# xiaochuanle/MECAT

Hardware: AMD Instinct MI355X
Metric: candidate overlaps/sec (higher is better)
Workload: dtype int32

## Files before the change

### mecat_amd/csrc/seed_cand.hip

```cpp
#include "seed_defs.h"
#include "seed_replay.h"

struct CandLds {
    int t_loc[2 * SM + 10];
    int t_seed[2 * SM + 10];
};

__device__ __forceinline__ int seg_find(const uint32_t* __restrict__ seg_id, int nseg, uint32_t seg) {
    int lo = 0, hi = nseg;
    while (lo < hi) {
        int mid = (lo + hi) >> 1;
        if (seg_id[mid] < seg) lo = mid + 1; else hi = mid;
    }
    return (lo < nseg && seg_id[lo] == seg) ? lo : -1;
}

__device__ __forceinline__ bool ddf_find(int dloc, int dseed, double cutoff) {
    float r = (float)dloc / ((float)dseed * 10.0f) - 1.0f;
    return (double)fabsf(r) < cutoff;
}

__device__ __forceinline__ bool ddf_find_quarter(int dloc, int dseed) {
    return (int)(2 * dloc > __mul24(15, dseed)) & (int)(2 * dloc < __mul24(25, dseed));
}

__device__ __forceinline__ int write_lane(int v, int l, int old) {
    asm volatile("s_mov_b32 m0, %2\n\tv_writelane_b32 %0, %1, m0" : "+v"(old) : "s"(v), "s"(l));
    return old;
}

__global__ __launch_bounds__(WAVE) __attribute__((amdgpu_waves_per_eu(7, 7))) void seed_cand(SeedArrays AF, SeedArrays AB, const mhip_offset_t* __restrict__ ref_offs, const uint32_t* __restrict__ ref_blk, int ref_nreads,
                                                  int ref_start_id, const mhip_offset_t* __restrict__ roffs, ReadSel sel, int ib,
                                                  int reads_start_id, mhip_params P, mhip_candidate* __restrict__ out,
                                                  int32_t* __restrict__ out_counts, unsigned long long* __restrict__ counters) {
    extern __shared__ __attribute__((aligned(16))) int smem[];
    const int lane = lane_id();
    const int r = blockIdx.x;
    const bool big = P.maxc > MAXC_LDS;
    int* clist = big ? (int*)(out + (size_t)r * P.maxc) : smem;
    CandLds* T = (CandLds*)(smem + (big ? 0 : P.maxc * 12));
    auto cl_ld = [&](int i) -> int { return big ? __hip_atomic_load(clist + i, __ATOMIC_RELAXED, __HIP_MEMORY_SCOPE_AGENT) : clist[i]; };
    auto cl_st = [&](int i, int v) { if (big) __hip_atomic_store(clist + i, v, __ATOMIC_RELAXED, __HIP_MEMORY_SCOPE_AGENT); else clist[i] = v; };
    const int rid = sel_rid(sel, ib + r);
    const int read_id = rid + reads_start_id;
    const int read_size = roffs[rid].size;
    const int MAXC = P.maxc;
    const double cutoff = P.ddfs_cutoff;
    int ncand = 0;

    for (int strand = 0; strand < 2; ++strand) {
        const int s = 2 * r + strand;
        const SeedArrays& A = AF.fused[s] ? AF : AB;
        const uint64_t hb = A.hit_base[s];
        const int nseg = (int)A.nseg[s];
        const int ng = (int)A.ngated[s];
        if (A.strand_hits[s] == 0) continue;
        uint32_t* ent = A.ent + hb;
        uint32_t* fin = A.ent_fin + hb;
        const uint32_t* seg_id = A.seg_id + hb;
        const uint32_t* seg_start = A.seg_start + hb;
        int32_t* seg_score = A.seg_score + hb;
        const uint32_t* gated = A.gated + hb;
#define SEG_LIST(g) (((seg_score[g] & OVF_FLAG) ? fin : ent) + seg_start[g])
#define SEG_SCORE(g) (seg_score[g] & ~OVF_FLAG)
#define SET_SCORE(g, v) seg_score[g] = (seg_score[g] & OVF_FLAG) | (v)

        int g_n = 0, seg_n = 0, segm1_n = -1;
        uint32_t st_n = 0, stm1_n = 0;
        auto prefetch = [&](int gi) {
            g_n = (int)gated[gi];
            seg_n = (int)seg_id[g_n];
            st_n = seg_start[g_n];
            segm1_n = g_n > 0 ? (int)seg_id[g_n - 1] : -1;
            stm1_n = g_n > 0 ? seg_start[g_n - 1] : 0u;
        };
        if (ng > 0) prefetch(0);
        for (int gi = 0; gi < ng; ++gi) {
            const int g = g_n, seg = seg_n, segm1 = segm1_n;
            const uint32_t st_g = st_n, st_gm1 = stm1_n;
            if (gi + 1 < ng) prefetch(gi + 1);
#ifdef CAND_STATS
            if (lane == 0) atomicAdd(&counters[9], 1ull);
#endif
            const int raw_g = seg_score[g];
            int s_k = raw_g & ~OVF_FLAG;
            if (s_k == 0) continue;
#ifdef CAND_STATS
            if (lane == 0) atomicAdd(&counters[10], 1ull);
#endif
            int start_loc = seg * ZV;
            int loc = 0, raw_gm1 = 0;
            const bool has_left = seg > 0 && g > 0 && segm1 == seg - 1;
            if (has_left) { raw_gm1 = seg_score[g - 1]; loc = raw_gm1 & ~OVF_FLAG; }
            if (loc > 0) start_loc = (seg - 1) * ZV;
            const int n1 = loc > 0 ? min(loc, SM) : 0, n2 = min(s_k, SM);
            const int k = n1 + n2;
            const uint32_t* list_g = ((raw_g & OVF_FLAG) ? fin : ent) + st_g;
            const uint32_t* list_gm1 = ((raw_gm1 & OVF_FLAG) ? fin : ent) + st_gm1;
            __syncthreads();
            for (int i = lane; i < k; i += 64) {
                uint32_t e = i < n1 ? list_gm1[i] : list_g[i - n1];
                T->t_loc[i] = ent_loc(e) + ((i >= n1 && loc > 0) ? ZV : 0);
                T->t_seed[i] = ent_seed(e);
            }
            __syncthreads();
            const int i0 = lane, i1 = lane + 64;
            const int l0 = i0 < k ? T->t_loc[i0] : 0, d0 = i0 < k ? T->t_seed[i0] : 0;
            const int l1 = i1 < k ? T->t_loc[i1] : 0, d1 = i1 < k ? T->t_seed[i1] : 0;
            int temp0 = d0, temp1 = d1, sc0 = 0, sc1 = 0;
            const int k0 = min(k, 64);
            int in0 = 0, in1 = 0;
            auto vote_loops = [&](auto ddf) {
                for (int j = 1; j < k0; ++j) {
                    const int lj = __builtin_amdgcn_readlane(l0, j), dj = __builtin_amdgcn_readlane(d0, j);
                    const int ds = dj - d0, dl = lj - l0;
                    const bool v0 = (i0 < j) & (temp0 != dj) & (ds > 0) & (dl > 0) & (dl < read_size) & ddf(dl, ds);
                    sc0 += v0 ? 1 : 0;
                    temp0 = v0 ? dj : temp0;
                    in0 = write_lane(__popcll(__builtin_amdgcn_ballot_w64(v0)), j, in0);
                }
                for (int j = 64; j < k; ++j) {
                    const int lj = __builtin_amdgcn_readlane(l1, j - 64), dj = __builtin_amdgcn_readlane(d1, j - 64);
                    const int ds0 = dj - d0, dl0 = lj - l0, ds1 = dj - d1, dl1 = lj - l1;
                    const bool v0 = (temp0 != dj) & (ds0 > 0) & (dl0 > 0) & (dl0 < read_size) & ddf(dl0, ds0);
                    const bool v1 = (i1 < j) & (temp1 != dj) & (ds1 > 0) & (dl1 > 0) & (dl1 < read_size) & ddf(dl1, ds1);
                    sc0 += v0 ? 1 : 0;
                    temp0 = v0 ? dj : temp0;
                    sc1 += v1 ? 1 : 0;
                    temp1 = v1 ? dj : temp1;
                    in1 = write_lane(__popcll(__builtin_amdgcn_ballot_w64(v0)) + __popcll(__builtin_amdgcn_ballot_w64(v1)), j - 64, in1);
                }
            };
            if (cutoff == 0.25) vote_loops([](int dloc, int dseed) { return ddf_find_quarter(dloc, dseed); });
            else vote_loops([&](int dloc, int dseed) { return (dloc > 0) & (dseed > 0) & ddf_find(dloc, dseed, cutoff); });
            sc0 += in0;
            sc1 += in1;
            int mv = max(i0 < k ? sc0 : -1, i1 < k ? sc1 : -1);
            for (int o = 32; o > 0; o >>= 1) mv = max(mv, __shfl_xor(mv, o));
            const int maxval = mv;
#ifdef CAND_STATS
            if (lane == 0 && maxval < 5) atomicAdd(&counters[11], 1ull);
            if (lane == 0) atomicAdd(&counters[12], (unsigned long long)k);
#endif
            if (maxval < 5) continue;
            const uint64_t eq0 = __ballot(i0 < k && sc0 == maxval), eq1 = __ballot(i1 < k && sc1 == maxval);
            const int maxi = eq0 ? __ffsll((unsigned long long)eq0) - 1 : 64 + __ffsll((unsigned long long)eq1) - 1;
            const int rep = __popcll(eq0) + __popcll(eq1) - 1;
            int rep_loc;
            if (rep == maxval) {
                rep_loc = maxi;
            } else {
                const int lm = T->t_loc[maxi], dm = T->t_seed[maxi];
                bool q0 = false, q1 = false;
                if (i0 < k) {
                    if (i0 < maxi) q0 = dm - d0 > 0 && lm - l0 > 0 && lm - l0 < read_size && ddf_find(lm - l0, dm - d0, cutoff);
                    else if (i0 == maxi) q0 = true;
                    else q0 = d0 - dm > 0 && l0 - lm > 0 && l0 - lm <= read_size && ddf_find(l0 - lm, d0 - dm, cutoff);
                }
                if (i1 < k) {
                    if (i1 < maxi) q1 = dm - d1 > 0 && lm - l1 > 0 && lm - l1 < read_size && ddf_find(lm - l1, dm - d1, cutoff);
                    else if (i1 == maxi) q1 = true;
                    else q1 = d1 - dm > 0 && l1 - lm > 0 && l1 - lm <= read_size && ddf_find(l1 - lm, d1 - dm, cutoff);
                }
                const uint64_t s0m = __ballot(q0), s1m = __ballot(q1);
                const uint64_t z0 = __ballot(q0 && l0 != 0), z1 = __ballot(q1 && l1 != 0);
                if (z0) rep_loc = __ffsll((unsigned long long)z0) - 1;
                else if (z1) rep_loc = 64 + __ffsll((unsigned long long)z1) - 1;
                else if (s1m) rep_loc = 64 + (63 - __clzll((unsigned long long)s1m));
                else rep_loc = 63 - __clzll((unsigned long long)s0m);
            }
            const int vote = rep_loc < 64 ? __shfl(sc0, rep_loc) : __shfl(sc1, rep_loc - 64);
            if (vote < 2 * P.min_kmer_match + 2) continue;
            const int loc_seed = T->t_seed[rep_loc];
            const int loc_list = start_loc + T->t_loc[rep_loc];
            int sid = read_id_lookup(ref_offs, ref_nreads, ref_blk, loc_list);
            const int sstart = ref_offs[sid].offset, ssize = ref_offs[sid].size;
            const int send = sstart + ssize + 1;
            sid += ref_start_id;
            if (sid > read_id) continue;
            if (sid == read_id) {
                int u_k = sstart / ZV;
                int gg = seg_find(seg_id, nseg, (uint32_t)u_k);
                if (gg >= 0) {
                    const int lim = sstart % ZV, cnt = min(SEG_SCORE(gg), SM);
                    uint32_t* L = SEG_LIST(gg);
                    uint32_t e = lane < cnt ? L[lane] : 0;
                    bool keep = lane < cnt && ent_loc(e) < lim;
                    uint64_t km = __ballot(keep);
                    int dstp = __popcll(km & ((1ull << lane) - 1ull));
                    __syncthreads();
                    if (keep) L[dstp] = (L[dstp] & 0xFFFFu) | (e & 0xFFFF0000u);
                    __syncthreads();
                    if (lane == 0) SET_SCORE(gg, __popcll(km));
                }
                ++u_k;
                const int kend = send / ZV;
                {
                    int lo = 0, hi = nseg;
                    while (lo < hi) { int mid = (lo + hi) >> 1; if ((int)seg_id[mid] < u_k) lo = mid + 1; else hi = mid; }
                    for (int x = lo + lane; x < nseg && (int)seg_id[x] < kend; x += 64) SET_SCORE(x, 0);
                }
                const int tail_seg = max(u_k, kend);
                gg = seg_find(seg_id, nseg, (uint32_t)tail_seg);
                __syncthreads();
                if (gg >= 0) {
                    const int lim = send % ZV, cnt = min(SEG_SCORE(gg), SM);
                    uint32_t* L = SEG_LIST(gg);
                    uint32_t e = lane < cnt ? L[lane] : 0;
                    bool keep = lane < cnt && ent_loc(e) > lim;
                    uint64_t km = __ballot(keep);
                    int dstp = __popcll(km & ((1ull << lane) - 1ull));
                    __syncthreads();
                    if (keep) L[dstp] = (L[dstp] & 0xFFFFu) | (e & 0xFFFF0000u);
                    __syncthreads();
                    if (lane == 0) SET_SCORE(gg, __popcll(km));
                }
                __syncthreads();
                continue;
            }
            const int loc2 = (loc_seed - 1) * BC;
            const int left1 = loc_list - sstart + MHIP_KMER_SIZE - 1, right1 = send - loc_list;
            const int left2 = loc2 + MHIP_KMER_SIZE - 1, right2 = read_size - loc2;
            const int num1 = left1 > left2 ? left2 : left1, num2 = right1 > right2 ? right2 : right1;
            if (num1 + num2 < P.min_kmer_dist) continue;
            int seedcount = 0;
            {
                int nlb = (num1 + ZV - 1) / ZV;
                const int lowest = max(0, seg - nlb);
                for (int x = g - 1; x >= 0 && (int)seg_id[x] >= lowest; --x) {
                    const int sc = SEG_SCORE(x);
                    if (sc <= 0) continue;
                    const int sl = (int)seg_id[x] * ZV, scnt = min(sc, SM);
                    bool ok = false;
                    if (lane < scnt) {
                        uint32_t e = SEG_LIST(x)[lane];
                        ok = fabs((double)(loc_list - sl - ent_loc(e)) / ((double)((loc_seed - ent_seed(e)) * BC) * 1.0) - 1.0) < cutoff;
                    }
                    const int agree = __popcll(__ballot(ok));
                    seedcount += agree;
                    if (agree * 1.0 / scnt > 0.4) { if (lane == 0) SET_SCORE(x, 0); }
                    __syncthreads();
                }
                int nrb = (num2 + ZV - 1) / ZV;
                const int highest = seg + nrb;
                for (int x = g + 1; x < nseg && (int)seg_id[x] <= highest; ++x) {
                    const int sc = SEG_SCORE(x);
                    if (sc <= 0) continue;
                    const int sl = (int)seg_id[x] * ZV, scnt = min(sc, SM);
                    bool ok = false;
                    if (lane < scnt) {
                        uint32_t e = SEG_LIST(x)[lane];
                        ok = fabs((double)(sl + ent_loc(e) - loc_list) / ((double)((ent_seed(e) - loc_seed) * BC) * 1.0) - 1.0) < cutoff;
                    }
                    const int agree = __popcll(__ballot(ok));
                    seedcount += agree;
                    if (agree * 1.0 / scnt > 0.4) { if (lane == 0) SET_SCORE(x, 0); }
                    __syncthreads();
                }
            }
            const int cscore = vote + seedcount;
            int ge = 0;
            for (int i = lane; i < ncand; i += 64) ge += cl_ld(i * 12 + 6) >= cscore ? 1 : 0;
            for (int o = 32; o > 0; o >>= 1) ge += __shfl_xor(ge, o);
            const int pos = ge;
            const int last_src = (ncand < MAXC) ? ncand - 1 : ncand - 2;
            __syncthreads();
            for (int top = last_src; top >= pos; top -= 64) {
                const int i = top - lane;
                int v[12];
                if (i >= pos) {
#pragma unroll
                    for (int q = 0; q < 12; ++q) v[q] = cl_ld(i * 12 + q);
                }
                __syncthreads();
                if (i >= pos) {
#pragma unroll
                    for (int q = 0; q < 12; ++q) cl_st((i + 1) * 12 + q, v[q]);
                }
                __syncthreads();
            }
            if (pos < MAXC && lane == 0) {
                const int cv[12] = {loc_list - sstart, loc2, left1, left2, right1, right2, cscore, num1, num2, sid, sstart, strand};
#pragma unroll
                for (int q = 0; q < 12; ++q) cl_st(pos * 12 + q, cv[q]);
            }
            if (ncand < MAXC) ++ncand;
            __syncthreads();
        }
#undef SEG_LIST
#undef SEG_SCORE
#undef SET_SCORE
    }
    __syncthreads();
    int* o = (int*)(out + (size_t)r * MAXC);
    if (!big)
        for (int i = lane; i < ncand * 12; i += 64) o[i] = clist[i];
    if (lane == 0) {
        out_counts[r] = ncand;
        atomicAdd(&counters[2], (unsigned long long)ncand);
    }
}

int seed_run_cand(const SeedBatch& b) {
    mhip_ctx* c = b.c;
    const mhip_params* P = b.P;
    const size_t lds = sizeof(int) * 12 * (size_t)(P->maxc > MAXC_LDS ? 0 : P->maxc) + sizeof(CandLds);
    LAUNCH(c, "seed_cand", seed_cand, b.nr, WAVE, lds, b.F, b.B, (const mhip_offset_t*)b.ref->d_offs, (const uint32_t*)b.ref->d_blk2read,
           b.ref->num_reads, b.ref->start_read_id, (const mhip_offset_t*)b.reads->d_offs, b.sel, b.ib, b.reads->start_read_id, *P, b.d_out,
           b.d_counts, (unsigned long long*)c->d_counters);
    return 0;
}
```

### mecat_amd/csrc/seed_replay.h

```cpp
#pragma once

#include "seed_defs.h"

__device__ __forceinline__ int sweep_reach(int L) { return (L + MHIP_KMER_SIZE - 1 + ZV - 1) / ZV + 1; }

__device__ __forceinline__ bool ddf_insert(int dloc, int dseed, double cutoff) {
    float r = (float)dloc / ((float)dseed * 10.0f);
    return fabs((double)r - 1.0) < cutoff;
}

__device__ void replay_overflow(const uint32_t* __restrict__ ev, int c, uint32_t* __restrict__ fin, uint16_t* __restrict__ esc,
                                double cutoff, int* score_out) {
    const int lane = lane_id();
    int loc = 0, seed = 0;
    if (lane < SM) { const uint32_t e0 = ev[lane]; loc = ent_loc(e0); seed = ent_seed(e0); }
    if (lane < SM) esc[lane] = (uint16_t)(lane + 1);
    int score = SM;
    int e = SM;
    auto is_chain = [&]() {
        const int nl = __shfl_down(loc, 1), ns = __shfl_down(seed, 1);
        return (bool)__all(lane >= SM - 1 || (ns - seed > 0 && nl - loc == (ns - seed) * BC));
    };
    bool chain = is_chain();
    while (e < c) {
        if (chain) {
            const int lloc = __builtin_amdgcn_readlane(loc, SM - 1), lseed = __builtin_amdgcn_readlane(seed, SM - 1);
            int nb = c;
            for (int i0 = e; i0 < c && nb == c; i0 += 64) {
                const int i = i0 + lane;
                bool bad = false;
                if (i < c) {
                    const uint32_t b = ev[i];
                    int pl = lloc, ps = lseed;
                    if (i > e) { const uint32_t a = ev[i - 1]; pl = ent_loc(a); ps = ent_seed(a); }
                    const int ds = ent_seed(b) - ps, dl = ent_loc(b) - pl;
                    bad = !(ds > 0 && dl == ds * BC);
                }
                const unsigned long long bm = __ballot(bad);
                if (bm) nb = i0 + __builtin_ctzll(bm);
            }
            if (nb > e) {
                for (int x = e + lane; x < nb; x += 64) esc[x] = (uint16_t)(score + (x - e) + 1);
                score += nb - e;
                if (lane == SM - 1) { const uint32_t le = ev[nb - 1]; loc = ent_loc(le); seed = ent_seed(le); }
                e = nb;
                if (e >= c) break;
            }
        }
        const uint32_t ne = ev[e];
        const int nloc = ent_loc(ne), nseed = ent_seed(ne);
        ++score;
        const int myloc = lane < SM ? loc : nloc, myseed = lane < SM ? seed : nseed;
        int sc = 0;
        for (int i = 0; i < SM; ++i) {
            const int li = __builtin_amdgcn_readlane(myloc, i), si = __builtin_amdgcn_readlane(myseed, i);
            const bool pass = lane > i && lane <= SM && myseed - si > 0 && myloc - li > 0 && ddf_insert(myloc - li, myseed - si, cutoff);
            const uint64_t b = __ballot(pass);
            sc += pass ? 1 : 0;
            if (lane == i) sc += __popcll(b);
        }
        const int v = lane <= SM ? sc : 0x7fffffff;
        int m = v;
        for (int o = 32; o > 0; o >>= 1) m = min(m, __shfl_xor(m, o));
        const int minval = m;
        const int mini = __ffsll((unsigned long long)__ballot(v == m)) - 1;
        if (minval == SM) {
            if (lane == SM - 1) { loc = nloc; seed = nseed; }
        } else if (minval < SM && mini < SM) {
            const int sl = __shfl_down(myloc, 1), ss = __shfl_down(myseed, 1);
            if (lane >= mini && lane < SM) { loc = sl; seed = ss; }
            --score;
        }
        if (lane == 0) esc[e] = (uint16_t)score;
        ++e;
        chain = is_chain();
    }
    if (lane < SM) fin[lane] = ((uint32_t)loc << 16) | ((uint32_t)seed & 0xFFFFu);
    *score_out = score;
}

__device__ __forceinline__ int read_id_from_offset(const mhip_offset_t* __restrict__ a, int n, int offset) {
    int left = 0, right = n - 1, mid = (left + right) / 2;
    if (a[right].offset < offset) return right;
    while (left <= right) {
        int o = a[mid].offset, z = a[mid].size;
        if (o <= offset && o + z > offset) return mid;
        if (o + z <= offset) left = mid + 1;
        else right = mid - 1;
        mid = (left + right) / 2;
    }
    return mid;
}

__device__ __forceinline__ int read_id_lookup(const mhip_offset_t* __restrict__ a, int n, const uint32_t* __restrict__ blk, int offset) {
    if (offset >= 0) {
        int r = (int)blk[offset >> 10];
        while (r + 1 < n && a[r].offset + a[r].size <= offset) ++r;
        const int o = a[r].offset, z = a[r].size;
        if (o <= offset && o + z > offset) return r;
    }
    return read_id_from_offset(a, n, offset);
}

__device__ __forceinline__ bool subjects_all_higher(const RefReads& R, uint32_t seg, int rid, int own_end) {
    const int lo = (int)((seg > 0 ? seg - 1u : 0u) * (uint32_t)ZV);
    if (R.same_volume) return lo >= own_end;
    return read_id_lookup(R.offs, R.nreads, R.blk, lo) + R.start_id > rid + R.reads_start_id;
}
```

Before: 7.212 million.

## Batch gated-segment metadata per wave and parallelize neighbor-segment sweep across lanes

```diff
diff --git a/mecat_amd/csrc/seed_cand.hip b/mecat_amd/csrc/seed_cand.hip
--- a/mecat_amd/csrc/seed_cand.hip
+++ b/mecat_amd/csrc/seed_cand.hip
@@ -1,5 +1,7 @@
 #include "seed_defs.h"
 #include "seed_replay.h"
+
+#define SWEEP_G 8
 
 struct CandLds {
     int t_loc[2 * SM + 10];
@@ -35,7 +37,7 @@
                                                   int32_t* __restrict__ out_counts, unsigned long long* __restrict__ counters) {
     extern __shared__ __attribute__((aligned(16))) int smem[];
     const int lane = lane_id();
-    const int r = blockIdx.x;
+    const int r = (int)gridDim.x - 1 - (int)blockIdx.x;
     const bool big = P.maxc > MAXC_LDS;
     int* clist = big ? (int*)(out + (size_t)r * P.maxc) : smem;
     CandLds* T = (CandLds*)(smem + (big ? 0 : P.maxc * 12));
@@ -64,34 +66,47 @@
 #define SEG_LIST(g) (((seg_score[g] & OVF_FLAG) ? fin : ent) + seg_start[g])
 #define SEG_SCORE(g) (seg_score[g] & ~OVF_FLAG)
 #define SET_SCORE(g, v) seg_score[g] = (seg_score[g] & OVF_FLAG) | (v)
-
-        int g_n = 0, seg_n = 0, segm1_n = -1;
-        uint32_t st_n = 0, stm1_n = 0;
-        auto prefetch = [&](int gi) {
-            g_n = (int)gated[gi];
-            seg_n = (int)seg_id[g_n];
-            st_n = seg_start[g_n];
-            segm1_n = g_n > 0 ? (int)seg_id[g_n - 1] : -1;
-            stm1_n = g_n > 0 ? seg_start[g_n - 1] : 0u;
-        };
-        if (ng > 0) prefetch(0);
+#define HAS_LEFT 0x40000000
+
+        int gv = 0, segv = 0, scv = 0, scm1v = 0;
+        uint32_t stv = 0, stm1v = 0;
+        bool stale = true;
         for (int gi = 0; gi < ng; ++gi) {
-            const int g = g_n, seg = seg_n, segm1 = segm1_n;
-            const uint32_t st_g = st_n, st_gm1 = stm1_n;
-            if (gi + 1 < ng) prefetch(gi + 1);
+            const int gj = gi & 63;
+            if (gj == 0) {
+                gv = segv = 0;
+                stv = stm1v = 0;
+                if (gi + lane < ng) {
+                    gv = (int)gated[gi + lane];
+                    segv = (int)seg_id[gv];
+                    stv = seg_start[gv];
+                    const int segm1 = gv > 0 ? (int)seg_id[gv - 1] : -1;
+                    if (segv > 0 && gv > 0 && segm1 == segv - 1) { segv |= HAS_LEFT; stm1v = seg_start[gv - 1]; }
+                }
+                stale = true;
+            }
+            if (stale) {
+                scv = scm1v = 0;
+                if (gi - gj + lane < ng) {
+                    scv = seg_score[gv];
+                    if (segv & HAS_LEFT) scm1v = seg_score[gv - 1];
+                }
+                stale = false;
+            }
 #ifdef CAND_STATS
             if (lane == 0) atomicAdd(&counters[9], 1ull);
 #endif
-            const int raw_g = seg_score[g];
+            const int raw_g = __builtin_amdgcn_readlane(scv, gj);
             int s_k = raw_g & ~OVF_FLAG;
             if (s_k == 0) continue;
 #ifdef CAND_STATS
             if (lane == 0) atomicAdd(&counters[10], 1ull);
 #endif
+            const int g = __builtin_amdgcn_readlane(gv, gj), seg = __builtin_amdgcn_readlane(segv, gj) & ~HAS_LEFT;
+            const uint32_t st_g = (uint32_t)__builtin_amdgcn_readlane((int)stv, gj), st_gm1 = (uint32_t)__builtin_amdgcn_readlane((int)stm1v, gj);
+            const int raw_gm1 = __builtin_amdgcn_readlane(scm1v, gj);
+            const int loc = raw_gm1 & ~OVF_FLAG;
             int start_loc = seg * ZV;
-            int loc = 0, raw_gm1 = 0;
-            const bool has_left = seg > 0 && g > 0 && segm1 == seg - 1;
-            if (has_left) { raw_gm1 = seg_score[g - 1]; loc = raw_gm1 & ~OVF_FLAG; }
             if (loc > 0) start_loc = (seg - 1) * ZV;
             const int n1 = loc > 0 ? min(loc, SM) : 0, n2 = min(s_k, SM);
             const int k = n1 + n2;
@@ -170,10 +185,11 @@
                 else rep_loc = 63 - __clzll((unsigned long long)s0m);
             }
             const int vote = rep_loc < 64 ? __shfl(sc0, rep_loc) : __shfl(sc1, rep_loc - 64);
+            const int loc_seed = __builtin_amdgcn_readfirstlane(T->t_seed[rep_loc]);
+            const int loc_list = start_loc + __builtin_amdgcn_readfirstlane(T->t_loc[rep_loc]);
+            const int blk_r = loc_list >= 0 ? (int)ref_blk[loc_list >> 10] : 0;
             if (vote < 2 * P.min_kmer_match + 2) continue;
-            const int loc_seed = T->t_seed[rep_loc];
-            const int loc_list = start_loc + T->t_loc[rep_loc];
-            int sid = read_id_lookup(ref_offs, ref_nreads, ref_blk, loc_list);
+            int sid = read_id_lookup_from(ref_offs, ref_nreads, blk_r, loc_list);
             const int sstart = ref_offs[sid].offset, ssize = ref_offs[sid].size;
             const int send = sstart + ssize + 1;
             sid += ref_start_id;
@@ -216,6 +232,7 @@
                     if (lane == 0) SET_SCORE(gg, __popcll(km));
                 }
                 __syncthreads();
+                stale = true;
                 continue;
             }
             const int loc2 = (loc_seed - 1) * BC;
@@ -225,38 +242,57 @@
             if (num1 + num2 < P.min_kmer_dist) continue;
             int seedcount = 0;
             {
-                int nlb = (num1 + ZV - 1) / ZV;
+                const int nlb = (num1 + ZV - 1) / ZV, nrb = (num2 + ZV - 1) / ZV;
                 const int lowest = max(0, seg - nlb);
-                for (int x = g - 1; x >= 0 && (int)seg_id[x] >= lowest; --x) {
-                    const int sc = SEG_SCORE(x);
-                    if (sc <= 0) continue;
-                    const int sl = (int)seg_id[x] * ZV, scnt = min(sc, SM);
-                    bool ok = false;
-                    if (lane < scnt) {
-                        uint32_t e = SEG_LIST(x)[lane];
-                        ok = fabs((double)(loc_list - sl - ent_loc(e)) / ((double)((loc_seed - ent_seed(e)) * BC) * 1.0) - 1.0) < cutoff;
+                const int highest = seg + nrb;
+                const bool lside = lane < 32;
+                uint64_t more = ~0ull;
+                for (int c = 0; more; ++c) {
+                    const int x = lside ? g - 1 - 32 * c - lane : g + 1 + 32 * c + (lane - 32);
+                    int id = -1, raw = 0;
+                    uint32_t st = 0;
+                    if (((more >> lane) & 1) && x >= 0 && x < nseg) { id = (int)seg_id[x]; raw = seg_score[x]; st = seg_start[x]; }
+                    const bool in = id >= 0 && (lside ? id >= lowest : id <= highest);
+                    const uint64_t inm = __builtin_amdgcn_ballot_w64(in);
+                    more = ((uint32_t)inm == 0xFFFFFFFFu ? 0xFFFFFFFFull : 0ull) | ((uint32_t)(inm >> 32) == 0xFFFFFFFFu ? 0xFFFFFFFF00000000ull : 0ull);
+                    const int scnt = min(raw & ~OVF_FLAG, SM);
+                    const uint64_t live = __builtin_amdgcn_ballot_w64(in && (raw & ~OVF_FLAG) > 0);
+                    int agv = 0;
+                    uint64_t m = live;
+                    while (m) {
+                        uint32_t e[SWEEP_G];
+                        uint64_t p = m;
+#pragma unroll
+                        for (int q = 0; q < SWEEP_G; ++q) {
+                            const bool has = p != 0;
+                            const int j = has ? __builtin_ctzll(p) : 0;
+                            p &= p - 1;
+                            const int rj = __builtin_amdgcn_readlane(raw, j);
+                            const uint32_t* L = ((rj & OVF_FLAG) ? fin : ent) + (uint32_t)__builtin_amdgcn_readlane((int)st, j);
+                            e[q] = 0;
+                            if (has && lane < min(rj & ~OVF_FLAG, SM)) e[q] = L[lane];
+                        }
+#pragma unroll
+                        for (int q = 0; q < SWEEP_G; ++q) {
+                            if (m) {
+                                const int j = __builtin_ctzll(m);
+                                m &= m - 1;
+                                const int sl = __builtin_amdgcn_readlane(id, j) * ZV, sc = __builtin_amdgcn_readlane(scnt, j);
+                                const int l = ent_loc(e[q]), sd = ent_seed(e[q]);
+                                const int dl = j < 32 ? loc_list - sl - l : sl + l - loc_list;
+                                const int ds = j < 32 ? loc_seed - sd : sd - loc_seed;
+                                const bool ok = lane < sc && fabs((double)dl / ((double)(ds * BC) * 1.0) - 1.0) < cutoff;
+                                const int agree = __popcll(__builtin_amdgcn_ballot_w64(ok));
+                                seedcount += agree;
+                                agv = write_lane(agree, j, agv);
+                            }
+                        }
                     }
-                    const int agree = __popcll(__ballot(ok));
-                    seedcount += agree;
-                    if (agree * 1.0 / scnt > 0.4) { if (lane == 0) SET_SCORE(x, 0); }
-                    __syncthreads();
-                }
-                int nrb = (num2 + ZV - 1) / ZV;
-                const int highest = seg + nrb;
-                for (int x = g + 1; x < nseg && (int)seg_id[x] <= highest; ++x) {
-                    const int sc = SEG_SCORE(x);
-                    if (sc <= 0) continue;
-                    const int sl = (int)seg_id[x] * ZV, scnt = min(sc, SM);
-                    bool ok = false;
-                    if (lane < scnt) {
-                        uint32_t e = SEG_LIST(x)[lane];
-                        ok = fabs((double)(sl + ent_loc(e) - loc_list) / ((double)((ent_seed(e) - loc_seed) * BC) * 1.0) - 1.0) < cutoff;
-                    }
-                    const int agree = __popcll(__ballot(ok));
-                    seedcount += agree;
-                    if (agree * 1.0 / scnt > 0.4) { if (lane == 0) SET_SCORE(x, 0); }
-                    __syncthreads();
-                }
+                    const bool zero = ((live >> lane) & 1) && agv * 1.0 / scnt > 0.4;
+                    if (zero) seg_score[x] = raw & OVF_FLAG;
+                    stale |= __builtin_amdgcn_ballot_w64(zero) != 0;
+                }
+                if (stale) __syncthreads();
             }
             const int cscore = vote + seedcount;
             int ge = 0;
@@ -290,6 +326,7 @@
 #undef SEG_LIST
 #undef SEG_SCORE
 #undef SET_SCORE
+#undef HAS_LEFT
     }
     __syncthreads();
     int* o = (int*)(out + (size_t)r * MAXC);
diff --git a/mecat_amd/csrc/seed_replay.h b/mecat_amd/csrc/seed_replay.h
--- a/mecat_amd/csrc/seed_replay.h
+++ b/mecat_amd/csrc/seed_replay.h
@@ -102,6 +102,15 @@
     return read_id_from_offset(a, n, offset);
 }
 
+__device__ __forceinline__ int read_id_lookup_from(const mhip_offset_t* __restrict__ a, int n, int r, int offset) {
+    if (offset >= 0) {
+        while (r + 1 < n && a[r].offset + a[r].size <= offset) ++r;
+        const int o = a[r].offset, z = a[r].size;
+        if (o <= offset && o + z > offset) return r;
+    }
+    return read_id_from_offset(a, n, offset);
+}
+
 __device__ __forceinline__ bool subjects_all_higher(const RefReads& R, uint32_t seg, int rid, int own_end) {
     const int lo = (int)((seg > 0 ? seg - 1u : 0u) * (uint32_t)ZV);
     if (R.same_volume) return lo >= own_end;
```

Result: faster. 7.291 million, median of 6 (+1.1%).
